# consensus-shipyard/ipc-filecoin-proofs

Measured on AMD Instinct MI355X. Metric: Merkle proofs verified/sec + HBM GB/s, 1M-receipt synthetic tipset, 1/2/4/8 GPU, higher is better.
Workload: dtype u64; 1 GPU; BASELINE.json configs[2] (the 1M-receipt tipset the metric is quoted on): 1000000 receipts (Amtv0<Receipt> + one Amt<...; receipts_per_gpu=1000000, claims_per_gpu=1000000, witness_blocks_per_gpu=1288038, witness_bytes_per_gpu=439923915, scan_matches=1002, device=AMD Radeon Graphics

## Files before the change

ipc-filecoin-proofs_amd/csrc/host/verify_fast.cpp:

```cpp
#include <chrono>
#include <cstdlib>
#include <cstring>
#include <memory>
#include <vector>

#include "../common.h"
#include "../kernels/claims_dev.h"
#include "../kernels/amt_enum.h"
#include "../kernels/event_table.h"
#include "../kernels/tipset_ctx.h"
#include "../kernels/types_dev.h"
#include "../kernels/launch.h"
#include "exec_state.h"

using namespace ipcfp;

namespace ipcfp {

int exec_state_prepare(ipcfp_ctx* ctx, ExecState& ex, uint32_t n_parents);

static int verify_packed_fast_queue(ipcfp_ctx* ctx, ipcfp_witness* w, std::vector<TipsetCtxDev>& tcs, const EventClaimPacked* claims_d,
                                    uint32_t n, const uint8_t* blob_d, uint64_t blob_len, const ipcfp_trust_policy_t* trust,
                                    const ipcfp_event_filter_t* filter, uint8_t* status_d, void* where_d, bool* done, ScanRide* ride);

// ... 64 lines not shown
    }
    ExecState ex;
    rc = exec_state_prepare(ctx, ex, P);
    if (rc) return rc;
    PrepareJob job{tcs_d.p, ex.roots.p, ex.err.p};
    DevBuf<EnumNode> frontier;
    DevBuf<DenseNode> dense_frontier;
    DevBuf<uint32_t> small_own;
    DevBuf<uint64_t> info_own;
    uint32_t* small = nullptr;
    uint64_t* info_d = nullptr;
    IPCFP_HIP(ctx, frontier.alloc(n_all));
    IPCFP_HIP(ctx, dense_frontier.alloc(n_all));
    IPCFP_HIP(ctx, ctl_words(ctx, small_own, small, 4, false));
    IPCFP_HIP(ctx, ctl_words(ctx, info_own, info_d, 2 * size_t(n_all), false));
    std::unique_ptr<ProfileScope> prof(new ProfileScope(ctx, IPCFP_K_TIPSET_PROLOGUE));
    const bool defer_rehash = !need_general && ctx->rehash_event != nullptr;
    rc = head ? launch_tipset_prepare(ctx, view, &job, nullptr, 1, false, w->index_done.p, w->index_wgs, small + 2, defer_rehash)
              : launch_tipset_prepare(ctx, view, &job, nullptr, 1, need_general, nullptr, 0, nullptr, defer_rehash,
                                      inline_inputs ? &inputs : nullptr);
    if (rc) return rc;
    if (head) {
        IPCFP_HIP(ctx, hipEventRecord(ctx->head_event, ctx->stream));
        IPCFP_HIP(ctx, hipStreamWaitEvent(swap.saved, ctx->head_event, 0));
        ctx->stream = swap.saved;
        for (auto& r : ctx->pending)
            if (r.stream == ctx->stream_head) r.stream = ctx->stream;
        if (prof) prof->stream = ctx->stream;
    }
    const unsigned long long seq = ++ctx->mailbox_seq;
    rc = launch_enum_roots(ctx, view, ex.roots.p, n_all, VK_CID, frontier.p, small, ex.err.p, info_d, ctx->mailbox_dev, seq,
                           dense_frontier.p);
    if (rc) return rc;
    prof.reset();
    {
        const auto deadline = std::chrono::steady_clock::now() + std::chrono::seconds(5);
        uint32_t spins = 0;
        while (__atomic_load_n(ctx->mailbox, __ATOMIC_ACQUIRE) != seq) {
            if ((++spins & 1023u) == 0 && std::chrono::steady_clock::now() > deadline) {
                IPCFP_HIP(ctx, sync_stream(ctx, ctx->stream));
                if (__atomic_load_n(ctx->mailbox, __ATOMIC_ACQUIRE) != seq)
                    return set_error(ctx, IPCFP_E_HIP, "the AMT roots' shapes never reached the mailbox");
            }
        }
    }
    std::vector<uint64_t> root_info(2 * size_t(n_all));
    for (size_t i = 0; i < root_info.size(); ++i) root_info[i] = __atomic_load_n(ctx->mailbox + 1 + i, __ATOMIC_RELAXED);
    DensePlan plan;
    dense_plan(root_info, n_roots, VK_CID, true, 0, ~0ULL, 1, VK_RECEIPT, w->receipt_lo, w->receipt_hi, plan);
    if (!plan.ok || plan.n_use != n_all || plan.n_leaves == 0 || plan.n_extra == 0) {
        IPCFP_HIP(ctx, sync_stream(ctx, ctx->stream));
        return IPCFP_OK;
    }
    const uint32_t n_msgs = uint32_t(plan.n_leaves), n_rcpt = uint32_t(plan.n_extra);
    DevBuf<DenseNode> a, b;
    DevBuf<LeafRef> rleaves;
    IPCFP_HIP(ctx, a.alloc(plan.biggest));
    IPCFP_HIP(ctx, b.alloc(plan.biggest));
    IPCFP_HIP(ctx, ex.keys.alloc(n_msgs));
    IPCFP_HIP(ctx, rleaves.alloc(n_rcpt));
    uint32_t size = 64;
    while (size < 2ull * n_msgs) size <<= 1;
    ex.mask = size - 1;
    ex.raw_len = n_msgs;
    IPCFP_HIP(ctx, ex.slots.alloc(size));
    const size_t first_words = (size_t(n_msgs) + 1) & ~size_t(1), scan_ctl_words = exec_scan_ctl_words(n_msgs);
    IPCFP_HIP(ctx, ex.first.alloc(first_words + 2 * scan_ctl_words));
    IPCFP_HIP(ctx, ex.pos.alloc(n_msgs));
    IPCFP_HIP(ctx, ex.inv.alloc(n_msgs));
    unsigned long long* const scan_ctl = reinterpret_cast<unsigned long long*>(ex.first.p + first_words);
    const DenseClear clear{ex.slots.p, size, ex.first.p, first_words + 2 * scan_ctl_words};
    std::unique_ptr<EventTableCached> table(new EventTableCached());
    table->lo = w->receipt_lo;
    table->hi = w->receipt_hi;
    table->n = n_rcpt;
    table->events = w->bt_events.p;
    IPCFP_HIP(ctx, table->receipts.alloc(n_rcpt));
    IPCFP_HIP(ctx, table->err_word.alloc(1));
    table->has_counts = w->bt_has_filter;
    if (table->has_counts) {
        table->counts_filter = w->bt_filter;
        IPCFP_HIP(ctx, table->counts.alloc(n_rcpt));
    }
    IPCFP_HIP(ctx, hipMemsetAsync(table->err_word.p, 0xff, 8, ctx->stream_aux));
    const DenseReceiptOut recs{w->bt_blocks.p, table->receipts.p, table->has_counts ? table->counts.p : nullptr, table->err_word.p};
    prof.reset(new ProfileScope(ctx, IPCFP_K_AMT_WALK));
    rc = launch_dense_walk(ctx, view, dense_frontier.p, plan, a.p, b.p, nullptr, ex.keys.p, rleaves.p, small + 2, ctx->stream_aux,
                           ctx->main_event, ctx->stream != swap.saved ? swap.saved : nullptr, ctx->narrow_event, ctx->narrow_max_wg,
                           &clear, &recs);
    if (rc) return rc;
    for (auto& r : ctx->pending)
        if (ctx->stream_narrow && r.stream == ctx->stream_narrow) r.stream = ctx->stream;
    if (prof) prof->stream = ctx->stream;
    prof.reset();
    if (ctx->k1_defer == 1 && (rc = k1_flush(ctx, true))) return rc;
    rc = launch_receipt_walk(ctx, view, rleaves.p, n_rcpt, table->has_counts ? &w->bt_filter.filter : nullptr,
                             int(w->bt_filter.has_actor), w->bt_filter.actor, table->receipts.p,
                             table->has_counts ? table->counts.p : nullptr, table->err_word.p, ctx->stream_aux);
    if (rc) return rc;
    IPCFP_HIP(ctx, hipEventRecord(ctx->aux_event, ctx->stream_aux));
    w->bt_joined = false;
    DevBuf<uint32_t> ride_counts, ride_offsets;
    DevBuf<unsigned long long> ride_err_own;
    unsigned long long ride_seq = 0;
    if (ride && ctx->scan_fused != 0 && ride->cap_matches <= (1ull << 26) && (!ride->has_d || ride->cap_receipts >= n_rcpt)) {
        struct OnAux {
            ipcfp_ctx* c;
            hipStream_t saved;
            ~OnAux() { c->stream = saved; }
        } on_aux{ctx, ctx->stream};
        ctx->stream = ctx->stream_aux;
        const ScanParams want = scan_params_of(ride->filter, ride->has_actor, ride->actor);
        const EventTableView tview = table->view();
        const uint32_t* cnt = nullptr;
        const unsigned long long* table_err = nullptr;
        unsigned long long* err_p = nullptr;
        IPCFP_HIP(ctx, ctl_words(ctx, ride_err_own, err_p, 1, true));
        if (table->has_counts && std::memcmp(&want, &table->counts_filter, sizeof want) == 0) {
            cnt = table->counts.p;
            table_err = table->err_word.p;
        } else {
            IPCFP_HIP(ctx, ride_counts.alloc(n_rcpt));
            rc = launch_count_from_table(ctx, view, rleaves.p, n_rcpt, ride->filter, ride->has_actor, ride->actor, tview, ride_counts.p, err_p);
            if (rc) return rc;
            cnt = ride_counts.p;
        }
        IPCFP_HIP(ctx, ride_offsets.alloc(n_rcpt));
        unsigned long long* tail_scratch = nullptr;
        rc = scan_tail_scratch(ctx, div_up(n_rcpt, 1024), &tail_scratch);
        if (rc) return rc;
        ride_seq = ++ctx->mailbox_seq;
        rc = launch_scan_tail_fused(ctx, view, rleaves.p, n_rcpt, w->receipt_lo, ride->filter, ride->has_actor, ride->actor, tview, cnt,
                                    ride_offsets.p, ride->cap_matches ? ride->matches_d : nullptr, ride->matches_d ? ride->cap_matches : 0,
                                    ride->has_d, ride->has_d ? n_rcpt : 0, w->receipt_lo, tail_scratch, ++ctx->scan_epoch, table_err,
                                    err_p, ctx->mailbox_dev, ride_seq);
        if (rc) return rc;
        ctx->scan_hint = want;
        ctx->has_scan_hint = true;
    }
    if (defer_rehash) {
        rc = launch_txmeta_rehash(ctx, ctx->stream_aux, view, tcs_d.p, ex.err.p);
        if (rc) return rc;
    }
    prof.reset(new ProfileScope(ctx, IPCFP_K_EXEC_ORDER));
    rc = launch_exec_insert_flags(ctx, ex.keys.p, n_msgs, ex.slots.p, ex.mask, ex.first.p);
    if (rc) return rc;
    IPCFP_HIP(ctx, ctl_words(ctx, ex.total_own, ex.total.p, 1, false));
    CtxFinish fin{};
    fin.err = ex.err.p;
    fin.total = ex.total.p;
    fin.first = ex.first.p;
    fin.pos = ex.pos.p;
    fin.inv = ex.inv.p;
    fin.slots = ex.slots.p;
    fin.keys = ex.keys.p;
    fin.mask = ex.mask;
    fin.raw_len = n_msgs;
    fin.receipt_leaves = rleaves.p;
    fin.n_receipt_leaves = n_rcpt;
    fin.receipt_first = w->receipt_lo;
    fin.receipt_recs = table->receipts.p;
    fin.event_recs = table->events;
    rc = launch_exec_scan_finish(ctx, tcs_d.p, fin, ex.pos.p, ex.total.p, scan_ctl);
    if (rc) return rc;
    prof.reset();
    rc = event_table_join(ctx, w);
    if (rc) return rc;
// ... 69 lines not shown
```

ipc-filecoin-proofs_amd/csrc/kernels/amt_enum.hip:

```cpp
#include "amt_enum.h"

#include <hip/hip_runtime.h>

#include <cstdlib>
#include <cstring>
#include <vector>

#include "../common.h"
#include "blake2b_dev.h"
#include "event_table.h"
#include "launch.h"
#include "tipset_ctx.h"

namespace ipcfp {

__device__ __forceinline__ void enum_error(unsigned long long* err, uint32_t seq, uint64_t base, uint32_t code) {
    atomicMin(err, (unsigned long long)pack_enum_error(seq, base, code));
}

__device__ __forceinline__ bool amt_load_dense_root(const WitnessView& w, const CidKey& root, int version, AmtRootInfo& info);

__device__ __forceinline__ void enum_root_one(const WitnessView& w, const AmtRootSpec& spec, int vkind, EnumNode* __restrict__ slot,
                                              uint32_t* __restrict__ max_height, unsigned long long* __restrict__ err,
                                              uint64_t& info0, uint64_t& info1, DenseNode* __restrict__ dense_slot) {
// ... 403 lines not shown
};
__device__ __forceinline__ DenseWhere dense_where(const DenseRoot* roots, uint32_t j, uint32_t level_here) {
    DenseWhere o;
    uint32_t r = 0;
    o.upper_off = o.here_off = 0;
    o.dr = roots[0];
    uint64_t n_here = dense_nodes(o.dr, level_here);
    while (j >= o.here_off + n_here) {
        o.here_off += uint32_t(n_here);
        o.upper_off += uint32_t(dense_nodes(o.dr, level_here + 1));
        o.dr = roots[++r];
        n_here = dense_nodes(o.dr, level_here);
    }
    return o;
}

__device__ __forceinline__ void dense_level_one(const WitnessView& w, const DenseNode* __restrict__ cur, const DenseRoot* roots,
                                                uint32_t level, uint32_t j, DenseNode* __restrict__ next,
                                                uint32_t* __restrict__ anomaly) {
    const DenseWhere wh = dense_where(roots, j, level - 1);
    const DenseRoot& dr = wh.dr;
    if (dr.height < level) {
        next[j] = cur[wh.upper_off];
        return;
    }
    const uint64_t q = dense_first(dr, level - 1) + (j - wh.here_off);
    const uint32_t W = 1u << dr.bit_width;
    const uint64_t p = q >> dr.bit_width;
    const uint32_t k = uint32_t(q) & (W - 1u);
    const DenseNode e = cur[wh.upper_off + uint32_t(p - dense_first(dr, level))];
    DenseNode c{0, e.base + uint64_t(k) * amt_span(dr.bit_width, level), kNoBlock, 0, e.seq, 1};
    if (e.block == kNoBlock) {
        next[j] = c;
        return;
    }
    const uint64_t remaining = dense_total(dr, level - 1) - p * W;
    const uint32_t m = remaining < W ? uint32_t(remaining) : W;
    const uint64_t n_here = dense_nodes(dr, level - 1);
    const bool edge_first = j == wh.here_off && k > 0;
    const bool edge_last = j + 1 == wh.here_off + n_here && k + 1 < m;
    uint64_t h0, h1;
    const uint32_t hdr = dense_header(W, m, false, h0, h1);
    const uint8_t* node = w.arena + e.goff;
    const uint32_t mine = hdr + 43u * k;
    bool ok = hdr != 0 && mine + 43u <= e.rem && header_matches(node, hdr, h0, h1) && std_link_at(node + mine);
    if (ok && edge_first)
        for (uint32_t i = 0; i < k && ok; ++i) ok = std_link_at(node + hdr + 43u * i);
    if (ok && edge_last)
        for (uint32_t i = k + 1; i < m && ok; ++i) ok = hdr + 43u * (i + 1u) <= e.rem && std_link_at(node + hdr + 43u * i);
    if (ok && (k == m - 1 || edge_last)) {
        const uint32_t tail = hdr + 43u * m;
        ok = tail + 1u <= e.rem && node[tail] == 0x80u && (!e.whole || tail + 1u == e.rem);
    }
    if (!ok) {
        atomicOr(anomaly, 1u);
        next[j] = c;
        return;
    }
    const CidKey key = std_link_key(node + mine);
    uint32_t s = cid_hash(key) & w.mask;
    for (;;) {
        const uint32_t b = w.slots[s];
        if (b == kNoBlock) {
            atomicOr(anomaly, 1u);
            break;
        }
        const CidKey have = load_cid_slot(w.cids, b);
        const uint64_t off = w.off[b];
        const uint32_t len = w.len[b];
        if (cid_equal(have, key)) {
            if (w.touched) atomicOr(&w.touched[b >> 5], 1u << (b & 31));
            c.block = b;
            c.goff = off;
            c.rem = len;
            break;
        }
        s = (s + 1) & w.mask;
    }
    next[j] = c;
}

__global__ __launch_bounds__(256) void k_dense_level(WitnessView w, const DenseNode* __restrict__ cur, const DenseRoots roots_arg,
                                                     uint32_t level, uint32_t n_next, DenseNode* __restrict__ next,
                                                     uint32_t* __restrict__ anomaly) {
    const uint32_t j = blockIdx.x * blockDim.x + threadIdx.x;
    if (j < n_next) dense_level_one(w, cur, roots_arg.r, level, j, next, anomaly);
}

struct DenseTopCounts {
    uint32_t n[8];
};
__global__ __launch_bounds__(256) void k_dense_top(WitnessView w, const DenseNode* frontier, const DenseRoots roots_arg, uint32_t level_hi,
                                                   uint32_t n_levels, DenseTopCounts counts, DenseNode* a, DenseNode* b,
                                                   uint32_t* __restrict__ anomaly) {
    const DenseNode* src = frontier;
    for (uint32_t i = 0; i < n_levels; ++i) {
        const uint32_t n_next = counts.n[i];
        for (uint32_t j = threadIdx.x; j < n_next; j += blockDim.x) dense_level_one(w, src, roots_arg.r, level_hi - i, j, a, anomaly);
        __syncthreads();
        src = a;
        DenseNode* t = a;
        a = b;
        b = t;
    }
}

__global__ __launch_bounds__(256) void k_dense_link_leaves(WitnessView w, const DenseNode* __restrict__ cur, const DenseRoots roots_arg,
                                                           uint32_t n_key_roots, uint64_t n_values, uint32_t* __restrict__ anomaly,
                                                           CidKey* __restrict__ keys_main, DenseClear clear) {
    const uint64_t v = uint64_t(blockIdx.x) * blockDim.x + threadIdx.x;
    {
        const uint64_t stride = uint64_t(gridDim.x) * blockDim.x;
        for (uint64_t j = v; j < clear.n_slots; j += stride) clear.slots[j] = ~0ull;
        for (uint64_t j = v; j < clear.n_words; j += stride) clear.words[j] = 0u;
    }
    if (v >= n_values) return;
    const DenseRoot* roots = roots_arg.r;
    uint32_t r = 0, node_off0 = 0;
    uint64_t voff = 0;
    DenseRoot dr = roots[0];
    while (r + 1 < n_key_roots && v >= voff + (dr.hi - dr.lo)) {
        voff += dr.hi - dr.lo;
        node_off0 += uint32_t(dense_nodes(dr, 0));
        dr = roots[++r];
    }
    const uint64_t idx = dr.lo + (v - voff);
    const uint32_t W = 1u << dr.bit_width;
    const uint64_t pnode = idx >> dr.bit_width;
    const uint32_t k = uint32_t(idx) & (W - 1u);
    const DenseNode e = cur[node_off0 + uint32_t(pnode - dense_first(dr, 0))];
    if (e.block == kNoBlock) return;
    const uint64_t remaining = dr.count - pnode * W;
    const uint32_t m = remaining < W ? uint32_t(remaining) : W;
    const bool edge_first = idx == dr.lo && k > 0;
    const bool edge_last = idx + 1 == dr.hi && k + 1 < m;
    uint64_t h0, h1;
    const uint32_t hdr = dense_header(W, m, true, h0, h1);
    const uint8_t* node = w.arena + e.goff;
    const uint32_t mine = hdr + 43u * k;
    bool ok = hdr != 0 && mine + 43u <= e.rem && header_matches(node, hdr, h0, h1) && std_link_at(node + mine);
    if (ok && edge_first)
        for (uint32_t i = 0; i < k && ok; ++i) ok = std_link_at(node + hdr + 43u * i);
    if (ok && edge_last)
        for (uint32_t i = k + 1; i < m && ok; ++i) ok = hdr + 43u * (i + 1u) <= e.rem && std_link_at(node + hdr + 43u * i);
    if (ok && (k == m - 1 || edge_last)) ok = !e.whole || hdr + 43u * m == e.rem;
    if (!ok) {
        atomicOr(anomaly, 1u);
        return;
    }
    keys_main[dr.out_off + (idx - dr.lo)] = std_link_key(node + mine);
}

__global__ __launch_bounds__(256) void k_dense_leaves(WitnessView w, const DenseNode* __restrict__ cur, const DenseRoots roots_arg,
                                                      uint32_t n_nodes, uint32_t first_node, LeafRef* __restrict__ leaves_main,
                                                      uint32_t* __restrict__ anomaly, LeafRef* __restrict__ leaves_extra) {
    const uint32_t t = first_node + blockIdx.x * blockDim.x + threadIdx.x;
    if (t >= n_nodes) return;
    const DenseWhere wh = dense_where(roots_arg.r, t, 0);
    const DenseRoot& dr = wh.dr;
    if (dr.out_sel == 0 && dr.count != 0) return;
    const uint64_t leaf_off = dr.out_off;
    const int vkind = int(dr.vkind);
    LeafRef* const leaves = dr.out_sel == 1 ? leaves_main : (dr.out_sel == 2 ? leaves_extra : nullptr);
    const uint64_t p = dense_first(dr, 0) + (t - wh.here_off);
    const DenseNode e = cur[t];
    const uint32_t W = 1u << dr.bit_width;
    const uint64_t remaining = dr.count - p * W;
    const uint32_t m = remaining < W ? uint32_t(remaining) : W;
    auto blank = [&]() {
        if (!leaves) return;
        for (uint32_t i = 0; i < m; ++i) {
            const uint64_t idx = p * W + i;
            if (idx >= dr.lo && idx < dr.hi) leaves[leaf_off + (idx - dr.lo)] = LeafRef{kNoBlock, 0, 0, e.seq, idx};
        }
    };
    if (e.block == kNoBlock) {
        blank();
        return;
    }
    const uint32_t node_off = uint32_t(e.goff - w.off[e.block]);
    Rd rd;
    rd.init(w.arena + e.goff, e.rem);
    rd.expect_array(3);
    uint32_t bo, bl;
    rd.read_bytes(bo, bl);
    bool ok = rd.ok() && bl == (W + 7) / 8;
    if (ok) {
        for (uint32_t i = 0; i < bl; ++i) {
            const uint32_t lo = i * 8u;
            uint32_t want = m >= lo + 8 ? 0xffu : (m > lo ? (1u << (m - lo)) - 1u : 0u);
            uint32_t have = rd.at(bo + i);
            if (W < 8) have &= (1u << W) - 1u;
            ok = ok && have == want;
        }
    }
    ok = ok && rd.read_array() == 0;
    const uint64_t nv = rd.read_array();
    ok = ok && rd.ok() && nv == m;
    for (uint32_t i = 0; ok && i < m; ++i) {
        const uint32_t start = rd.pos;
        const uint64_t idx = p * W + i;
        check_value(rd, vkind);
        ok = rd.ok();
        if (ok && leaves && idx >= dr.lo && idx < dr.hi)
            leaves[leaf_off + (idx - dr.lo)] = LeafRef{e.block, node_off + start, rd.pos - start, e.seq, e.base + i};
    }
    if (ok && e.whole) {
        rd.finish();
        ok = rd.ok();
    }
    if (!ok) {
        atomicOr(anomaly, 1u);
        blank();
    }
}

__device__ __forceinline__ uint32_t receipt_end_fast(const uint8_t* node, uint32_t s, uint32_t rem) {
    if (s >= rem) return 0;
    const uint64_t a0 = load_u64_any(node + s), a1 = load_u64_any(node + s + 8), a2 = load_u64_any(node + s + 16);
    auto ab = [&](uint32_t i) { return uint32_t((i < 8u ? a0 >> (8u * i) : (i < 16u ? a1 >> (8u * (i - 8u)) : a2 >> (8u * (i - 16u)))) & 0xffull); };
    auto extra = [](uint32_t info) { return info < 24u ? 0u : (info == 24u ? 1u : (info == 25u ? 2u : (info == 26u ? 4u : (info == 27u ? 8u : 99u)))); };
    if (ab(0) != 0x84u) return 0;
    uint32_t b = ab(1);
    uint32_t x = extra(b & 31u);
    if ((b >> 5) != 0u || x > 8u) return 0;
    uint32_t p = 2u + x;
    b = ab(p);
    x = extra(b & 31u);
    if ((b >> 5) != 2u || x > 4u) return 0;
    uint64_t len = b & 31u;
    if (x == 1u) len = ab(p + 1u);
    else if (x == 2u) len = (ab(p + 1u) << 8) | ab(p + 2u);
    else if (x == 4u) len = (uint64_t(ab(p + 1u)) << 24) | (ab(p + 2u) << 16) | (ab(p + 3u) << 8) | ab(p + 4u);
    const uint64_t g = uint64_t(s) + p + 1u + x + len;
    if (g >= rem) return 0;
    const uint64_t c0 = load_u64_any(node + g), c1 = load_u64_any(node + g + 8);
    auto cb = [&](uint32_t i) { return uint32_t((i < 8u ? c0 >> (8u * i) : c1 >> (8u * (i - 8u))) & 0xffull); };
    b = cb(0);
    x = extra(b & 31u);
    if ((b >> 5) != 0u || x > 8u) return 0;
    const uint32_t q = 1u + x;
    uint64_t end;
    if (cb(q) == 0xf6u) {
        end = g + q + 1u;
    } else {
        if (cb(q) != 0xd8u || cb(q + 1u) != 0x2au) return 0;
        b = cb(q + 2u);
        if ((b >> 5) != 2u || (b & 31u) > 24u) return 0;
        end = (b & 31u) < 24u ? g + q + 3u + (b & 31u) : g + q + 4u + cb(q + 3u);
    }
    return end <= rem ? uint32_t(end) : 0u;
}

__global__ __launch_bounds__(256) void k_dense_receipt_leaves(WitnessView w, const DenseNode* __restrict__ cur, const DenseRoots roots_arg,
                                                              uint32_t root_i, uint32_t node_off0, uint32_t n_values,
                                                              uint32_t* __restrict__ anomaly, LeafRef* __restrict__ leaves,
                                                              DenseReceiptOut out) {
    const uint32_t t = blockIdx.x * blockDim.x + threadIdx.x;
    if (t >= n_values) return;
    const DenseRoot dr = roots_arg.r[root_i];
    const uint64_t idx = dr.lo + t;
    const uint32_t W = 1u << dr.bit_width;
    const uint64_t pnode = idx >> dr.bit_width;
    const uint32_t k = uint32_t(idx) & (W - 1u);
    const DenseNode e = cur[node_off0 + uint32_t(pnode - dense_first(dr, 0))];
    const uint64_t remaining = dr.count - pnode * W;
    const uint32_t m = remaining < W ? uint32_t(remaining) : W;
    LeafRef lr{kNoBlock, 0, 0, e.seq, idx};
    ReceiptRec rr{RK_WALK, 0, 0, kNoBlock, 0};
    uint32_t c = 0;
    if (e.block != kNoBlock) {
        uint64_t h0, h1;
        const uint32_t hdr = dense_header(W, m, true, h0, h1);
        const uint8_t* node = w.arena + e.goff;
        bool ok = hdr != 0 && hdr < e.rem && k < m && header_matches(node, hdr, h0, h1);
        Rd rd;
        rd.init(node, e.rem);
        rd.pos = hdr;
        const bool check_before = idx == dr.lo && k > 0;
        for (uint32_t i = 0; ok && i < k; ++i) {
            const uint32_t end = check_before ? 0u : receipt_end_fast(node, rd.pos, e.rem);
            if (end) {
                rd.pos = end;
            } else {
                check_value(rd, VK_RECEIPT);
                ok = rd.ok();
            }
        }
        const uint32_t start = rd.pos;
        CidKey ev_root;
        bool has_root = false;
        if (ok) {
            rd.expect_array(4);
            if (rd.read_uint() > 0xffffffffULL) rd.fail();
            uint32_t o, l;
            rd.read_bytes(o, l);
            (void)rd.read_uint();
            if (rd.at_null()) rd.read_null();
            else has_root = rd.read_link_key(ev_root);
            ok = rd.ok();
        }
        const uint32_t stop = rd.pos;
        if (ok) {
            const uint32_t fast = receipt_end_fast(node, start, e.rem);
            ok = fast == 0u || fast == stop;
        }
        if (ok && (k + 1u == m || idx + 1u == dr.hi)) {
            for (uint32_t i = k + 1u; ok && i < m; ++i) {
                check_value(rd, VK_RECEIPT);
                ok = rd.ok();
            }
            if (ok && e.whole) {
                rd.finish();
                ok = rd.ok();
            }
        }
        if (!ok) {
            atomicOr(anomaly, 1u);
        } else {
            lr = LeafRef{e.block, uint32_t(e.goff - w.off[e.block]) + start, stop - start, e.seq, e.base + k};
            rr.kind = RK_NO_EVENTS;
            if (has_root) {
                const uint32_t b = witness_find(w, ev_root);
                rr.block = b;
                if (b == kNoBlock) {
                    rr.kind = IPCFP_ST_ERR_MISSING_BLOCK;
                    atomicMin(out.err, (unsigned long long)pack_enum_error(1, t, rr.kind));
                } else {
                    const BlockRec br = out.brecs[b];
                    if ((br.kind_matches & 0xffu) == RK_TABLE) {
                        rr.kind = RK_TABLE;
                        rr.first = br.first;
                        rr.bitmap = br.bitmap;
                        c = br.kind_matches >> 8;
                    } else {
                        rr.kind = RK_WALK;
                        c = kWalkPending;
                    }
                }
            }
        }
    }
    leaves[dr.out_off + t] = lr;
    out.rrecs[t] = rr;
    if (out.counts) out.counts[t] = c;
}

__global__ void k_enum_check(const uint64_t* __restrict__ actual, uint64_t expected, uint32_t* __restrict__ mismatch) {
    if (threadIdx.x == 0 && blockIdx.x == 0 && *actual != expected) atomicOr(mismatch, 1u);
}

int launch_scan_u32(ipcfp_ctx* ctx, const uint32_t* in_d, uint32_t n, uint32_t* out_d, uint64_t* total_d,
                    uint64_t* scratch_d);

static uint64_t predicted_frontier(const std::vector<uint64_t>& info, uint32_t level, uint32_t max_height) {
    if (level == max_height) return info.size() / 2;
    uint64_t total = 0;
    for (size_t i = 0; i + 1 < info.size(); i += 2) {
        if (info[i] == ~0ULL) continue;
        const uint32_t h = uint32_t(info[i]), bw = uint32_t(info[i] >> 32);
        const uint64_t c = info[i + 1];
        if (h <= level || c == 0) {
            total += 1;
        } else {
            const uint64_t shift = uint64_t(bw) * (level + 1);
            total += shift >= 64 ? 1 : ((c + (1ULL << shift) - 1) >> shift);
        }
    }
    return total;
}

static uint64_t amt_span_host(uint32_t bw, uint64_t height) {
    const uint64_t shift = uint64_t(bw) * height;
    return shift >= 64 ? ~0ULL : (1ULL << shift);
}

void dense_plan(const std::vector<uint64_t>& root_info, uint32_t n_roots, int vkind, bool want_keys, uint64_t lo, uint64_t hi,
                uint32_t has_extra, int extra_vkind, uint64_t extra_lo, uint64_t extra_hi, DensePlan& plan) {
    plan = DensePlan{};
    const uint32_t n_all = n_roots + (has_extra ? 1u : 0u);
    if (n_roots == 0 || n_all > kMaxDenseRoots || root_info.size() < 2 * size_t(n_all)) return;
    auto shape = [&](uint32_t i, uint64_t rlo, uint64_t rhi, DenseRoot& d) -> bool {
        if (root_info[2 * size_t(i)] == ~0ULL) return false;
        d.height = uint32_t(root_info[2 * size_t(i)]);
        d.bit_width = uint32_t(root_info[2 * size_t(i)] >> 32);
        d.count = root_info[2 * size_t(i) + 1];
        if (d.count == 0 && d.height > 0) return false;
        if (d.count > amt_span_host(d.bit_width, d.height + 1)) return false;
        d.lo = rlo < d.count ? rlo : d.count;
        d.hi = rhi < d.count ? rhi : d.count;
        if (d.count && d.lo >= d.hi) return false;
        if (d.count == 0) d.lo = d.hi = 0;
        return true;
    };
    bool try_dense = true;
    uint64_t n_leaves = 0;
    for (uint32_t i = 0; i < n_roots && try_dense; ++i) {
        try_dense = shape(i, lo, hi, plan.roots.r[i]);
        plan.roots.r[i].vkind = uint32_t(vkind);
        plan.roots.r[i].out_sel = want_keys ? 0u : 1u;
        plan.roots.r[i].out_off = n_leaves;
        n_leaves += plan.roots.r[i].hi - plan.roots.r[i].lo;
    }
    uint32_t n_use = n_roots;
    uint64_t n_extra = 0;
    if (has_extra && try_dense && shape(n_roots, extra_lo, extra_hi, plan.roots.r[n_roots])) {
        plan.roots.r[n_roots].vkind = uint32_t(extra_vkind);
        plan.roots.r[n_roots].out_sel = 2u;
        plan.roots.r[n_roots].out_off = 0;
        n_extra = plan.roots.r[n_roots].hi - plan.roots.r[n_roots].lo;
        n_use = n_all;
    }
    if (!try_dense) return;
    uint32_t max_height = 0;
    for (uint32_t i = 0; i < n_use; ++i) max_height = plan.roots.r[i].height > max_height ? plan.roots.r[i].height : max_height;
    if (max_height >= kMaxDenseLevels) return;
    uint64_t biggest = n_use;
    for (uint32_t level = 0; level <= max_height; ++level) {
        uint64_t nl = 0;
        for (uint32_t i = 0; i < n_use; ++i) nl += dense_nodes(plan.roots.r[i], level);
        if (nl >= 0x7fffffffULL) return;
        plan.n_level[level] = nl;
        biggest = nl > biggest ? nl : biggest;
    }
    if (n_leaves >= 0x7fffffffULL || n_extra >= 0x7fffffffULL || plan.n_level[max_height] != n_use) return;
    plan.ok = true;
    plan.n_use = n_use;
    plan.roots.n = n_use;
    plan.max_height = max_height;
    plan.n_leaves = n_leaves;
    plan.n_extra = n_extra;
    plan.biggest = biggest;
}

int launch_dense_walk(ipcfp_ctx* ctx, const WitnessView& view, const DenseNode* frontier, const DensePlan& plan,
                      DenseNode* a, DenseNode* b, LeafRef* leaves_main, CidKey* keys_main, LeafRef* leaves_extra, uint32_t* anomaly_d,
                      hipStream_t leaves_stream, hipEvent_t fork_event, hipStream_t wide_stream, hipEvent_t wide_event,
                      uint32_t narrow_max_wg, const DenseClear* clear, const DenseReceiptOut* receipts) {
    const DenseNode* src = frontier;
    auto widen = [&]() -> hipError_t {
        if (!wide_stream || ctx->stream == wide_stream) return hipSuccess;
        hipError_t e = hipEventRecord(wide_event, ctx->stream);
        if (e == hipSuccess) e = hipStreamWaitEvent(wide_stream, wide_event, 0);
        ctx->stream = wide_stream;
        return e;
    };
    uint32_t level_from = plan.max_height;
    {
        static const uint32_t top_max = [] {
            const char* e = std::getenv("IPCFP_DENSE_TOP");
            return e ? uint32_t(std::atoi(e)) : kDenseTopMax;
        }();
        DenseTopCounts counts{};
        uint32_t n_top = 0;
        while (n_top < 8 && level_from - n_top >= 1 && plan.n_level[level_from - n_top - 1] <= top_max) {
            counts.n[n_top] = uint32_t(plan.n_level[level_from - n_top - 1]);
            ++n_top;
        }
        if (n_top >= 2) {
            hipLaunchKernelGGL(k_dense_top, dim3(1), dim3(256), 0, ctx->stream, view, src, plan.roots, level_from, n_top, counts, a, b, anomaly_d);
            if (n_top & 1u) {
                src = a;
                DenseNode* t = a;
                a = b;
                b = t;
            } else {
                src = b;
            }
            level_from -= n_top;
        }
    }
    for (uint32_t level = level_from; level >= 1; --level) {
        const uint32_t nn = uint32_t(plan.n_level[level - 1]);
        if (div_up(nn, 256) > narrow_max_wg) IPCFP_HIP(ctx, widen());
        hipLaunchKernelGGL(k_dense_level, dim3(div_up(nn, 256)), dim3(256), 0, ctx->stream, view, src, plan.roots, level, nn, a, anomaly_d);
        src = a;
        DenseNode* t = a;
        a = b;
        b = t;
    }
    uint32_t n_key_roots = 0, key_nodes = 0;
    uint64_t n_key_values = 0;
    while (n_key_roots < plan.n_use && plan.roots.r[n_key_roots].out_sel == 0) {
        n_key_values += plan.roots.r[n_key_roots].hi - plan.roots.r[n_key_roots].lo;
        key_nodes += uint32_t(dense_nodes(plan.roots.r[n_key_roots], 0));
        ++n_key_roots;
    }
    for (uint32_t i = n_key_roots; i < plan.n_use; ++i)
        if (plan.roots.r[i].out_sel == 0) return set_error(ctx, IPCFP_E_INVALID, "dense walk: the key trees must come first");
    IPCFP_HIP(ctx, widen());
    hipStream_t ls = ctx->stream;
    if (leaves_stream && leaves_stream != ctx->stream && fork_event) {
        IPCFP_HIP(ctx, hipEventRecord(fork_event, ctx->stream));
        IPCFP_HIP(ctx, hipStreamWaitEvent(leaves_stream, fork_event, 0));
        ls = leaves_stream;
    }
    const uint32_t n_nodes = uint32_t(plan.n_level[0]);
    if (receipts) {
        const uint32_t ri = plan.n_use - 1;
        const DenseRoot& rr = plan.roots.r[ri];
        if (ri < n_key_roots || rr.out_sel != 2 || rr.vkind != VK_RECEIPT || !leaves_extra)
            return set_error(ctx, IPCFP_E_INVALID, "dense walk: the receipt records want a receipts tree as the extra root");
        const uint32_t r_nodes = uint32_t(dense_nodes(rr, 0)), before = n_nodes - r_nodes;
        bool node_lanes = ri > n_key_roots;
        for (uint32_t i = 0; i < n_key_roots; ++i) node_lanes = node_lanes || plan.roots.r[i].count == 0;
        if (node_lanes)
            hipLaunchKernelGGL(k_dense_leaves, dim3(div_up(before, 256)), dim3(256), 0, ls, view, src, plan.roots, before, 0u,
                               leaves_main, anomaly_d, nullptr);
        const uint32_t n_values = uint32_t(rr.hi - rr.lo);
        if (n_values)
            hipLaunchKernelGGL(k_dense_receipt_leaves, dim3(div_up(n_values, 256)), dim3(256), 0, ls, view, src, plan.roots, ri,
                               before, n_values, anomaly_d, leaves_extra, *receipts);
        else
            hipLaunchKernelGGL(k_dense_leaves, dim3(div_up(r_nodes, 256)), dim3(256), 0, ls, view, src, plan.roots, n_nodes, before,
                               leaves_main, anomaly_d, leaves_extra);
    } else {
        hipLaunchKernelGGL(k_dense_leaves, dim3(div_up(n_nodes, 256)), dim3(256), 0, ls, view, src, plan.roots, n_nodes, 0u,
                           leaves_main, anomaly_d, leaves_extra);
    }
    (void)key_nodes;
    if (clear && !n_key_values) {
        if (clear->n_slots) IPCFP_HIP(ctx, hipMemsetAsync(clear->slots, 0xff, clear->n_slots * 8, ctx->stream));
        if (clear->n_words) IPCFP_HIP(ctx, hipMemsetAsync(clear->words, 0, clear->n_words * 4, ctx->stream));
    }
    if (n_key_values)
        hipLaunchKernelGGL(k_dense_link_leaves, dim3(div_up(n_key_values, 256)), dim3(256), 0, ctx->stream, view, src, plan.roots,
                           n_key_roots, n_key_values, anomaly_d, keys_main, clear ? *clear : DenseClear{nullptr, 0, nullptr, 0});
    IPCFP_HIP(ctx, hipGetLastError());
    return IPCFP_OK;
}

int amt_enumerate(ipcfp_ctx* ctx, const WitnessView& view, const AmtRootSpec* roots_d, uint32_t n_roots, int vkind,
                  unsigned long long* err_d, AmtEnumResult& out, uint64_t lo, uint64_t hi, DevBuf<CidKey>* keys_out,
                  EnumExtra* extra) {
    out.keys_written = false;
    if (extra) {
        extra->done = false;
        if (!extra->out || n_roots == 0) extra = nullptr;
    }
    const uint32_t n_all = n_roots + (extra ? 1u : 0u);
    const EnumRange rg{lo, hi};
    const bool whole = lo == 0 && hi == ~0ULL;
    out.n_leaves = 0;
    out.error = kNoEnumError;
    out.leaves.release();
    if (n_roots == 0) return IPCFP_OK;
    ProfileScope prof(ctx, IPCFP_K_EXEC_ORDER);
    DevBuf<EnumNode> cur, nxt;
    DevBuf<uint32_t> counts, offsets, small_own;
    DevBuf<uint64_t> scratch, total_d, root_info_own;
    DevBuf<DenseNode> dense_cur;
    IPCFP_HIP(ctx, cur.alloc(n_all));
    IPCFP_HIP(ctx, dense_cur.alloc(n_all));
    IPCFP_HIP(ctx, total_d.alloc(2));
    uint32_t* small = nullptr;
    uint64_t* root_info_d = nullptr;
    IPCFP_HIP(ctx, ctl_words(ctx, small_own, small, 4, false));
    IPCFP_HIP(ctx, ctl_words(ctx, root_info_own, root_info_d, 2 * size_t(n_all), false));
    hipLaunchKernelGGL(k_enum_roots, dim3(div_up(n_all, 64)), dim3(64), 0, ctx->stream, view, roots_d, n_all, vkind,
                       cur.p, small, err_d, root_info_d, static_cast<unsigned long long*>(nullptr), 0ull, dense_cur.p);
    uint32_t max_height = 0;
    std::vector<uint64_t> root_info(2 * size_t(n_all));
    IPCFP_HIP(ctx, ctl_read(ctx, &max_height, small, 4));
    IPCFP_HIP(ctx, ctl_read(ctx, root_info.data(), root_info_d, root_info.size() * 8));
    IPCFP_HIP(ctx, sync_stream(ctx, ctx->stream));

    out.dense = false;
    {
        const bool want_keys = keys_out && vkind == VK_CID;
        DensePlan plan;
        dense_plan(root_info, n_roots, vkind, want_keys, lo, hi, extra ? 1u : 0u, extra ? extra->vkind : 0, extra ? extra->lo : 0,
                   extra ? extra->hi : 0, plan);
        if (plan.ok) {
            const uint32_t n_use = plan.n_use;
            DevBuf<DenseNode> a, b;
            struct { uint32_t* p; } anomaly{small + 2};
            IPCFP_HIP(ctx, a.alloc(plan.biggest));
            IPCFP_HIP(ctx, b.alloc(plan.biggest));
            if (want_keys) IPCFP_HIP(ctx, keys_out->alloc(plan.n_leaves));
            else IPCFP_HIP(ctx, out.leaves.alloc(plan.n_leaves));
            if (n_use > n_roots) IPCFP_HIP(ctx, extra->out->leaves.alloc(plan.n_extra));
            int rc = launch_dense_walk(ctx, view, dense_cur.p, plan, a.p, b.p, want_keys ? nullptr : out.leaves.p,
                                       want_keys ? keys_out->p : nullptr, n_use > n_roots ? extra->out->leaves.p : nullptr, anomaly.p);
            if (rc) return rc;
            uint32_t bad = 0;
            unsigned long long e = kNoEnumError;
            IPCFP_HIP(ctx, ctl_read(ctx, &bad, anomaly.p, 4));
            IPCFP_HIP(ctx, ctl_read(ctx, &e, err_d, 8));
            IPCFP_HIP(ctx, sync_stream(ctx, ctx->stream));
            IPCFP_HIP(ctx, hipGetLastError());
            if (!bad) {
                out.n_leaves = plan.n_leaves;
                out.error = e;
                out.dense = true;
                out.keys_written = want_keys;
                if (n_use > n_roots) {
// ... 245 lines not shown
```

Baseline: 1.151 billion proofs/s.

## Restructure receipt leaf walk: one thread group per node with LDS staging

```diff
diff --git a/ipc-filecoin-proofs_amd/csrc/host/verify_fast.cpp b/ipc-filecoin-proofs_amd/csrc/host/verify_fast.cpp
--- a/ipc-filecoin-proofs_amd/csrc/host/verify_fast.cpp
+++ b/ipc-filecoin-proofs_amd/csrc/host/verify_fast.cpp
@@ -170,7 +170,6 @@
         table->counts_filter = w->bt_filter;
         IPCFP_HIP(ctx, table->counts.alloc(n_rcpt));
     }
-    IPCFP_HIP(ctx, hipMemsetAsync(table->err_word.p, 0xff, 8, ctx->stream_aux));
     const DenseReceiptOut recs{w->bt_blocks.p, table->receipts.p, table->has_counts ? table->counts.p : nullptr, table->err_word.p};
     prof.reset(new ProfileScope(ctx, IPCFP_K_AMT_WALK));
     rc = launch_dense_walk(ctx, view, dense_frontier.p, plan, a.p, b.p, nullptr, ex.keys.p, rleaves.p, small + 2, ctx->stream_aux,
diff --git a/ipc-filecoin-proofs_amd/csrc/kernels/amt_enum.hip b/ipc-filecoin-proofs_amd/csrc/kernels/amt_enum.hip
--- a/ipc-filecoin-proofs_amd/csrc/kernels/amt_enum.hip
+++ b/ipc-filecoin-proofs_amd/csrc/kernels/amt_enum.hip
@@ -509,8 +509,9 @@
 
 __global__ __launch_bounds__(256) void k_dense_level(WitnessView w, const DenseNode* __restrict__ cur, const DenseRoots roots_arg,
                                                      uint32_t level, uint32_t n_next, DenseNode* __restrict__ next,
-                                                     uint32_t* __restrict__ anomaly) {
+                                                     uint32_t* __restrict__ anomaly, unsigned long long* __restrict__ set_err) {
     const uint32_t j = blockIdx.x * blockDim.x + threadIdx.x;
+    if (set_err && j == 0) *set_err = kNoEnumError;
     if (j < n_next) dense_level_one(w, cur, roots_arg.r, level, j, next, anomaly);
 }
 
@@ -519,7 +520,8 @@
 };
 __global__ __launch_bounds__(256) void k_dense_top(WitnessView w, const DenseNode* frontier, const DenseRoots roots_arg, uint32_t level_hi,
                                                    uint32_t n_levels, DenseTopCounts counts, DenseNode* a, DenseNode* b,
-                                                   uint32_t* __restrict__ anomaly) {
+                                                   uint32_t* __restrict__ anomaly, unsigned long long* __restrict__ set_err) {
+    if (set_err && threadIdx.x == 0) *set_err = kNoEnumError;
     const DenseNode* src = frontier;
     for (uint32_t i = 0; i < n_levels; ++i) {
         const uint32_t n_next = counts.n[i];
@@ -642,16 +644,18 @@
     }
 }
 
-__device__ __forceinline__ uint32_t receipt_end_fast(const uint8_t* node, uint32_t s, uint32_t rem) {
+template <class F8>
+__device__ __forceinline__ uint32_t receipt_value_fast(const F8& f8, uint32_t s, uint32_t rem, bool& root) {
+    root = false;
     if (s >= rem) return 0;
-    const uint64_t a0 = load_u64_any(node + s), a1 = load_u64_any(node + s + 8), a2 = load_u64_any(node + s + 16);
-    auto ab = [&](uint32_t i) { return uint32_t((i < 8u ? a0 >> (8u * i) : (i < 16u ? a1 >> (8u * (i - 8u)) : a2 >> (8u * (i - 16u)))) & 0xffull); };
+    const uint64_t a0 = f8(s), a1 = f8(s + 8u);
+    auto ab = [&](uint32_t i) { return uint32_t((i < 8u ? a0 >> (8u * i) : a1 >> (8u * (i - 8u))) & 0xffull); };
     auto extra = [](uint32_t info) { return info < 24u ? 0u : (info == 24u ? 1u : (info == 25u ? 2u : (info == 26u ? 4u : (info == 27u ? 8u : 99u)))); };
     if (ab(0) != 0x84u) return 0;
     uint32_t b = ab(1);
     uint32_t x = extra(b & 31u);
-    if ((b >> 5) != 0u || x > 8u) return 0;
-    uint32_t p = 2u + x;
+    if ((b >> 5) != 0u || x > 4u) return 0;
+    const uint32_t p = 2u + x;
     b = ab(p);
     x = extra(b & 31u);
     if ((b >> 5) != 2u || x > 4u) return 0;
@@ -661,90 +665,148 @@
     else if (x == 4u) len = (uint64_t(ab(p + 1u)) << 24) | (ab(p + 2u) << 16) | (ab(p + 3u) << 8) | ab(p + 4u);
     const uint64_t g = uint64_t(s) + p + 1u + x + len;
     if (g >= rem) return 0;
-    const uint64_t c0 = load_u64_any(node + g), c1 = load_u64_any(node + g + 8);
-    auto cb = [&](uint32_t i) { return uint32_t((i < 8u ? c0 >> (8u * i) : c1 >> (8u * (i - 8u))) & 0xffull); };
-    b = cb(0);
+    const uint64_t c0 = f8(uint32_t(g)), c1 = f8(uint32_t(g) + 8u), c2 = f8(uint32_t(g) + 16u);
+    auto cw = [&](uint32_t i) {
+        const uint32_t sh = 8u * (i & 7u);
+        const uint64_t lo = i < 8u ? c0 : (i < 16u ? c1 : c2), hi = i < 8u ? c1 : (i < 16u ? c2 : 0ull);
+        return sh ? (lo >> sh) | (hi << (64u - sh)) : lo;
+    };
+    b = uint32_t(c0 & 0xffu);
     x = extra(b & 31u);
     if ((b >> 5) != 0u || x > 8u) return 0;
     const uint32_t q = 1u + x;
+    const uint64_t t0 = cw(q);
     uint64_t end;
-    if (cb(q) == 0xf6u) {
+    if ((t0 & 0xffu) == 0xf6u) {
         end = g + q + 1u;
     } else {
-        if (cb(q) != 0xd8u || cb(q + 1u) != 0x2au) return 0;
-        b = cb(q + 2u);
-        if ((b >> 5) != 2u || (b & 31u) > 24u) return 0;
-        end = (b & 31u) < 24u ? g + q + 3u + (b & 31u) : g + q + 4u + cb(q + 3u);
+        if (t0 != 0xa071010027582ad8ull || (cw(q + 8u) & 0xffffffull) != 0x2002e4ull) return 0;
+        end = g + q + 43u;
+        root = true;
     }
     return end <= rem ? uint32_t(end) : 0u;
 }
 
-__global__ __launch_bounds__(256) void k_dense_receipt_leaves(WitnessView w, const DenseNode* __restrict__ cur, const DenseRoots roots_arg,
-                                                              uint32_t root_i, uint32_t node_off0, uint32_t n_values,
-                                                              uint32_t* __restrict__ anomaly, LeafRef* __restrict__ leaves,
-                                                              DenseReceiptOut out) {
-    const uint32_t t = blockIdx.x * blockDim.x + threadIdx.x;
-    if (t >= n_values) return;
-    const DenseRoot dr = roots_arg.r[root_i];
-    const uint64_t idx = dr.lo + t;
-    const uint32_t W = 1u << dr.bit_width;
-    const uint64_t pnode = idx >> dr.bit_width;
-    const uint32_t k = uint32_t(idx) & (W - 1u);
-    const DenseNode e = cur[node_off0 + uint32_t(pnode - dense_first(dr, 0))];
+constexpr uint32_t kReceiptStageBytes = 64;
+constexpr uint32_t kReceiptStageSlack = 6;
+__host__ __device__ inline uint32_t receipt_leaf_group(uint32_t bit_width) { return bit_width >= 6u ? 64u : (1u << bit_width); }
+__host__ __device__ inline uint32_t receipt_stage_words(uint32_t G) { return G * (kReceiptStageBytes / 8u) + kReceiptStageSlack; }
+
+__global__ __launch_bounds__(256) void k_dense_receipt_leaves(WitnessView w, const DenseNode* __restrict__ cur, const DenseRoot dr,
+                                                              uint32_t node_off0, uint32_t n_nodes, uint32_t* __restrict__ anomaly,
+                                                              LeafRef* __restrict__ leaves, DenseReceiptOut out) {
+    extern __shared__ uint64_t receipt_stage[];
+    const uint32_t W = 1u << dr.bit_width, G = receipt_leaf_group(dr.bit_width);
+    const uint32_t gid = (blockIdx.x * blockDim.x + threadIdx.x) / G, j = threadIdx.x & (G - 1u);
+    if (gid >= n_nodes) return;
+    uint64_t* const st = receipt_stage + (threadIdx.x / G) * receipt_stage_words(G);
+    const uint64_t pnode = dense_first(dr, 0) + gid;
+    const DenseNode e = cur[node_off0 + gid];
     const uint64_t remaining = dr.count - pnode * W;
     const uint32_t m = remaining < W ? uint32_t(remaining) : W;
-    LeafRef lr{kNoBlock, 0, 0, e.seq, idx};
-    ReceiptRec rr{RK_WALK, 0, 0, kNoBlock, 0};
-    uint32_t c = 0;
-    if (e.block != kNoBlock) {
-        uint64_t h0, h1;
-        const uint32_t hdr = dense_header(W, m, true, h0, h1);
-        const uint8_t* node = w.arena + e.goff;
-        bool ok = hdr != 0 && hdr < e.rem && k < m && header_matches(node, hdr, h0, h1);
+    uint64_t h0, h1;
+    const uint32_t hdr = dense_header(W, m, true, h0, h1);
+    const bool live = e.block != kNoBlock;
+    bool ok = live && hdr != 0 && hdr < e.rem;
+    const uint8_t* node = w.arena + e.goff;
+    const uint32_t sh = uint32_t(e.goff & 15u);
+    const bool staged = ok && e.rem <= G * kReceiptStageBytes - 16u;
+    if (staged) {
+        const ulonglong2* src = reinterpret_cast<const ulonglong2*>(node - sh);
+        const uint32_t n_ch = (sh + e.rem + 15u) / 16u;
+        ulonglong2 v[kReceiptStageBytes / 16u];
+#pragma unroll
+        for (uint32_t i = 0; i < kReceiptStageBytes / 16u; ++i)
+            if (j + G * i < n_ch) v[i] = src[j + G * i];
+#pragma unroll
+        for (uint32_t i = 0; i < kReceiptStageBytes / 16u; ++i)
+            if (j + G * i < n_ch) {
+                st[2u * (j + G * i)] = v[i].x;
+                st[2u * (j + G * i) + 1u] = v[i].y;
+            }
+        __builtin_amdgcn_fence(__ATOMIC_RELEASE, "wavefront");
+        __builtin_amdgcn_wave_barrier();
+        __builtin_amdgcn_fence(__ATOMIC_ACQUIRE, "wavefront");
+    }
+    const auto f8_stage = [&](uint32_t i) __attribute__((always_inline)) {
+        const uint32_t q = sh + i, r = 8u * (q & 7u);
+        const uint64_t lo = st[q >> 3], hi = st[(q >> 3) + 1u];
+        return r ? (lo >> r) | (hi << (64u - r)) : lo;
+    };
+    const auto f8_global = [&](uint32_t i) __attribute__((always_inline)) { return load_u64_any(node + i); };
+    uint32_t start = 0, stop = 0;
+    bool mine_fast = false, mine_root = false;
+    const auto pass = [&](const auto& f8) __attribute__((always_inline)) {
+        const uint64_t g0 = f8(0u), g1 = f8(8u);
+        const uint64_t m0 = hdr >= 8 ? ~0ull : ((1ull << (8u * hdr)) - 1ull);
+        const uint64_t m1 = hdr <= 8 ? 0ull : (hdr >= 16 ? ~0ull : ((1ull << (8u * (hdr - 8u))) - 1ull));
+        ok = ((g0 ^ h0) & m0) == 0 && ((g1 ^ h1) & m1) == 0;
         Rd rd;
         rd.init(node, e.rem);
-        rd.pos = hdr;
-        const bool check_before = idx == dr.lo && k > 0;
-        for (uint32_t i = 0; ok && i < k; ++i) {
-            const uint32_t end = check_before ? 0u : receipt_end_fast(node, rd.pos, e.rem);
-            if (end) {
-                rd.pos = end;
-            } else {
+        uint32_t pos = hdr;
+        for (uint32_t i = 0; ok && i < m; ++i) {
+            bool root;
+            uint32_t end = receipt_value_fast(f8, pos, e.rem, root);
+            const bool fast = end != 0u;
+            if (!fast) {
+                rd.pos = pos;
                 check_value(rd, VK_RECEIPT);
                 ok = rd.ok();
+                end = rd.pos;
             }
-        }
-        const uint32_t start = rd.pos;
-        CidKey ev_root;
-        bool has_root = false;
-        if (ok) {
+            if (i == j) {
+                start = pos;
+                stop = end;
+                mine_fast = fast;
+                mine_root = root;
+            }
+            pos = end;
+        }
+        if (ok && e.whole) ok = pos == e.rem;
+    };
+    if (staged) pass(f8_stage);
+    else if (ok) pass(f8_global);
+    if (live && !ok) atomicOr(anomaly, 1u);
+    CidKey ev_root;
+    bool has_root = false;
+    if (ok && j < m) {
+        if (mine_fast) {
+            has_root = mine_root;
+            if (has_root) {
+#pragma unroll
+                for (int q = 0; q < 5; ++q) ev_root.w[q] = staged ? f8_stage(stop - 38u + 8u * q) : f8_global(stop - 38u + 8u * q);
+                ev_root.w[4] &= (1ull << 48) - 1ull;
+            }
+        } else {
+            Rd rd;
+            rd.init(node, e.rem);
+            rd.pos = start;
             rd.expect_array(4);
             if (rd.read_uint() > 0xffffffffULL) rd.fail();
             uint32_t o, l;
             rd.read_bytes(o, l);
             (void)rd.read_uint();
-            if (rd.at_null()) rd.read_null();
-            else has_root = rd.read_link_key(ev_root);
-            ok = rd.ok();
-        }
-        const uint32_t stop = rd.pos;
-        if (ok) {
-            const uint32_t fast = receipt_end_fast(node, start, e.rem);
-            ok = fast == 0u || fast == stop;
-        }
-        if (ok && (k + 1u == m || idx + 1u == dr.hi)) {
-            for (uint32_t i = k + 1u; ok && i < m; ++i) {
-                check_value(rd, VK_RECEIPT);
-                ok = rd.ok();
+            if (rd.at_null()) {
+                rd.read_null();
+            } else {
+                uint32_t co, cl;
+                rd.read_link(co, cl);
+                if (cl > 40u) rd.fail();
+                has_root = rd.ok();
+                if (has_root) ev_root = rd.key_at(co, cl);
             }
-            if (ok && e.whole) {
-                rd.finish();
-                ok = rd.ok();
-            }
-        }
-        if (!ok) {
-            atomicOr(anomaly, 1u);
-        } else {
+            ok = rd.ok() && rd.pos == stop;
+            if (!ok) atomicOr(anomaly, 1u);
+        }
+    }
+    for (uint32_t k = j; k < m; k += G) {
+        const uint64_t idx = pnode * W + k;
+        if (idx < dr.lo || idx >= dr.hi) continue;
+        const uint32_t t = uint32_t(idx - dr.lo);
+        LeafRef lr{kNoBlock, 0, 0, e.seq, idx};
+        ReceiptRec rr{RK_WALK, 0, 0, kNoBlock, 0};
+        uint32_t c = 0;
+        if (ok && k == j) {
             lr = LeafRef{e.block, uint32_t(e.goff - w.off[e.block]) + start, stop - start, e.seq, e.base + k};
             rr.kind = RK_NO_EVENTS;
             if (has_root) {
@@ -767,10 +829,10 @@
                 }
             }
         }
-    }
-    leaves[dr.out_off + t] = lr;
-    out.rrecs[t] = rr;
-    if (out.counts) out.counts[t] = c;
+        leaves[dr.out_off + t] = lr;
+        out.rrecs[t] = rr;
+        if (out.counts) out.counts[t] = c;
+    }
 }
 
 __global__ void k_enum_check(const uint64_t* __restrict__ actual, uint64_t expected, uint32_t* __restrict__ mismatch) {
@@ -873,6 +935,7 @@
         return e;
     };
     uint32_t level_from = plan.max_height;
+    unsigned long long* set_err = receipts ? receipts->err : nullptr;
     {
         static const uint32_t top_max = [] {
             const char* e = std::getenv("IPCFP_DENSE_TOP");
@@ -885,7 +948,9 @@
             ++n_top;
         }
         if (n_top >= 2) {
-            hipLaunchKernelGGL(k_dense_top, dim3(1), dim3(256), 0, ctx->stream, view, src, plan.roots, level_from, n_top, counts, a, b, anomaly_d);
+            hipLaunchKernelGGL(k_dense_top, dim3(1), dim3(256), 0, ctx->stream, view, src, plan.roots, level_from, n_top, counts, a, b, anomaly_d,
+                               set_err);
+            set_err = nullptr;
             if (n_top & 1u) {
                 src = a;
                 DenseNode* t = a;
@@ -900,7 +965,9 @@
     for (uint32_t level = level_from; level >= 1; --level) {
         const uint32_t nn = uint32_t(plan.n_level[level - 1]);
         if (div_up(nn, 256) > narrow_max_wg) IPCFP_HIP(ctx, widen());
-        hipLaunchKernelGGL(k_dense_level, dim3(div_up(nn, 256)), dim3(256), 0, ctx->stream, view, src, plan.roots, level, nn, a, anomaly_d);
+        hipLaunchKernelGGL(k_dense_level, dim3(div_up(nn, 256)), dim3(256), 0, ctx->stream, view, src, plan.roots, level, nn, a, anomaly_d,
+                           set_err);
+        set_err = nullptr;
         src = a;
         DenseNode* t = a;
         a = b;
@@ -916,6 +983,7 @@
     for (uint32_t i = n_key_roots; i < plan.n_use; ++i)
         if (plan.roots.r[i].out_sel == 0) return set_error(ctx, IPCFP_E_INVALID, "dense walk: the key trees must come first");
     IPCFP_HIP(ctx, widen());
+    if (set_err) IPCFP_HIP(ctx, hipMemsetAsync(set_err, 0xff, sizeof *set_err, ctx->stream));
     hipStream_t ls = ctx->stream;
     if (leaves_stream && leaves_stream != ctx->stream && fork_event) {
         IPCFP_HIP(ctx, hipEventRecord(fork_event, ctx->stream));
@@ -934,11 +1002,12 @@
         if (node_lanes)
             hipLaunchKernelGGL(k_dense_leaves, dim3(div_up(before, 256)), dim3(256), 0, ls, view, src, plan.roots, before, 0u,
                                leaves_main, anomaly_d, nullptr);
-        const uint32_t n_values = uint32_t(rr.hi - rr.lo);
-        if (n_values)
-            hipLaunchKernelGGL(k_dense_receipt_leaves, dim3(div_up(n_values, 256)), dim3(256), 0, ls, view, src, plan.roots, ri,
-                               before, n_values, anomaly_d, leaves_extra, *receipts);
-        else
+        if (rr.hi > rr.lo) {
+            const uint32_t G = receipt_leaf_group(rr.bit_width);
+            hipLaunchKernelGGL(k_dense_receipt_leaves, dim3(div_up(uint64_t(r_nodes) * G, 256)), dim3(256),
+                               (256u / G) * receipt_stage_words(G) * sizeof(uint64_t), ls, view, src, rr, before, r_nodes, anomaly_d,
+                               leaves_extra, *receipts);
+        } else
             hipLaunchKernelGGL(k_dense_leaves, dim3(div_up(r_nodes, 256)), dim3(256), 0, ls, view, src, plan.roots, n_nodes, before,
                                leaves_main, anomaly_d, leaves_extra);
     } else {
```

Result: faster. 1.216 billion proofs/s (median of 6 runs) (+5.7%).
